# auggiemarignier/pxmcmc

Measured on AMD Instinct MI355X. Metric: MYULA samples/sec at L=256 synthesis, higher is better.
Workload: dtype f64

## Files before the change

pxmcmc_amd/csrc/sht_core.h:

```cpp
#pragma once
#include "common.h"

namespace pxm {

enum TableKind { TAB_INV = 0, TAB_FWD = 1, TAB_INV_ADJ = 2, TAB_FWD_ADJ = 3, TAB_GRAM = 4, TAB_GRAM_SPLIT = 5, TAB_KINDS = 6 };
inline bool kind_el_to_ring(int kind) { return kind == TAB_INV || kind == TAB_FWD_ADJ; }
inline bool kind_is_gram(int kind) { return kind == TAB_GRAM || kind == TAB_GRAM_SPLIT; }
inline bool kind_rows_are_el(int kind) { return kind == TAB_FWD || kind == TAB_INV_ADJ || kind_is_gram(kind); }
inline bool kind_k_is_el(int kind) { return kind == TAB_INV || kind == TAB_FWD_ADJ || kind_is_gram(kind); }

struct GemmTask {
  int64_t tab_off;
  int64_t rt_stride;
  int64_t x_off[4];
  int64_t y_off[4];
  int64_t x2_off[4];
  int64_t hd_off[4];
  int64_t ks_off[2];
  int64_t rs_off[2];
  int row_lo[2], row_hi[2];
  int k_beg, k_end;
  int row0;
  int n_rt;
  int nslab;
  double sign1;
  int m_unit;
  int hd_stride;
  int x_ncol, y_ncol;
};

struct GemmAffine {
  double ns = 0, wr = 0, wi = 0;
  int on = 0;
  int ncol_live = 1 << 30;
  uint64_t* bump = nullptr;
};

struct Profiler {
  struct Pool {
    std::vector<std::pair<hipEvent_t, hipEvent_t>> ev;
    size_t used = 0;
    double bytes = 0, flops = 0;
    std::vector<double> launch_bytes;
    std::vector<int> launch_wgs;
  };
  bool on = false;
  Pool gemm, dft;
  void next(Pool& p, hipEvent_t* start, hipEvent_t* stop, double alg_bytes, double flops, int workgroups = 0) {
    *start = *stop = nullptr;
    if (!on || p.used >= p.ev.size()) return;
    *start = p.ev[p.used].first;
// ... 9 lines not shown
int profiler_read(Profiler::Pool* p, double* ms, int64_t* launches, double* bytes, double* flops,
                  double* per_launch_ms = nullptr, double* per_launch_bytes = nullptr, int64_t cap = 0,
                  int32_t* per_launch_wgs = nullptr);
void profiler_release(Profiler* pr);

struct GemmFuse {
  int64_t x2_base = -1;
  const double* rscale = nullptr;
  int row_lo = 0, row_hi = 1 << 30;
  int64_t hd_base = -1;
  int hd_stride = 0;
};

struct ShtTables {
  int L = 0, spin = 0, Rp = 0;
  bool paired = false;
  int n_m = 0;
  double* d_tab[TAB_KINDS] = {};
  size_t bytes[TAB_KINDS] = {};
  std::vector<int64_t> m_off[TAB_KINDS];
  std::vector<int> k_beg[TAB_KINDS];
  std::vector<int64_t> odd_off;
  std::vector<int> odd_k_beg;
  int refs = 0;
  int m_of(int i) const { return paired ? i : i - (L - 1); }
};

inline bool gram_can_split(const ShtTables& T) { return T.paired && T.Rp % 32 == 0; }
constexpr int GEMM_TASK_FIXED_STEPS = 32;
inline int gram_half_k_beg(int m, int par) { return round_down((m - par + 1) / 2, 16); }
inline bool gram_order_splits(int Rp, int m) {
  auto work = [](int n, int kb) { return (n - kb) / 16 * (n - kb + GEMM_TASK_FIXED_STEPS); };
  return work(Rp / 2, gram_half_k_beg(m, 0)) + work(Rp / 2, gram_half_k_beg(m, 1)) < work(Rp, round_down(m, 16));
}

int get_tables(int L, int spin, unsigned kinds_mask, ShtTables** out);
void retain_tables(ShtTables* T);
void release_tables(ShtTables* T);
int64_t tables_trim();

void append_gemm_tasks(const ShtTables& T, int kind, int ncol, int64_t x_base, int x_L, int x_Rp,
                       int64_t y_base, int y_L, int y_Rp, const double* kscale, int64_t scratch_off,
                       const double* ws_base, std::vector<GemmTask>& tasks, int el_lo = 0,
                       const GemmFuse& fuse = GemmFuse());
struct GemmSide {
  int64_t x_base, y_base;
// ... 132 lines not shown
```

pxmcmc_amd/csrc/sht_gemm.hip:

```cpp
#include "../../include/pxmcmc_amd.h"
#include "sht_core.h"

#include <type_traits>

#include <hip/hip_ext.h>

#include <cstdlib>
#include <map>
#include <mutex>

namespace pxm {

typedef double d4 __attribute__((ext_vector_type(4)));

constexpr int KC = 16;
#define PXM_GEMM_MFMA(ACC, A, B) ACC = __builtin_amdgcn_mfma_f64_16x16x4f64(A, B, ACC, 0, 0, 0);
#ifdef PXM_GEMM_TRACE
__device__ unsigned long long* g_gemm_trace = nullptr;
extern "C" int pxm_debug_set_gemm_trace(unsigned long long* buf) {
  return hipMemcpyToSymbol(HIP_SYMBOL(g_gemm_trace), &buf, sizeof(buf)) == hipSuccess ? 0 : -1;
}
#endif
__device__ __forceinline__ double stage_add(double a, double b, bool on) { return a + (on ? b : 0.0); }
__device__ __forceinline__ double2 stage_add(double2 a, double2 b, bool on) { return double2{a.x + (on ? b.x : 0.0), a.y + (on ? b.y : 0.0)}; }
__device__ __forceinline__ double stage_scale(double a, double sc) { return a * sc; }
__device__ __forceinline__ double2 stage_scale(double2 a, double sc) { return double2{a.x * sc, a.y * sc}; }
template <int CT, int NSLAB>
struct GemmGeom {
  static constexpr int NCT = CT * NSLAB;
  static constexpr int COLS = 16 * NCT;
  static constexpr int PITCH = COLS + (COLS == 16 ? 0 : 16);
};
template <int CT, int NSLAB, int NW, int RT, int NSET, bool TWO, bool SK, int PK = 0>
__device__ __forceinline__ void sht_gemm_body(const GemmTask* __restrict__ tasks, const int bid,
                                              const double* __restrict__ X, double* __restrict__ Y, int ncol, int col0,
                                              const GemmAffine& aff, double (*xs)[KC][GemmGeom<CT, NSLAB>::PITCH]) {
  constexpr int NCT = CT * NSLAB;
  constexpr bool HOIST = TWO;
  constexpr int COLS = GemmGeom<CT, NSLAB>::COLS;
  constexpr int PITCH = GemmGeom<CT, NSLAB>::PITCH;
  constexpr int NT = 64 * NW;
  constexpr int VW = (KC * COLS / 2 >= NT) ? 2 : 1;
  constexpr int NV = KC * COLS / VW;
  constexpr int IT = (NV + NT - 1) / NT;
  const GemmTask t = tasks[bid];
  const int tid = threadIdx.x, lane = tid & 63;
  if (t.n_rt == 0) return;
  const int xn = (PK || TWO) ? t.x_ncol : ncol, yn = (PK || TWO) ? t.y_ncol : ncol;
#ifdef PXM_GEMM_TRACE
  const unsigned long long trace_t0 = wall_clock64();
  unsigned long long trace_t1 = 0, trace_t2 = 0;
  long long trace_c[5] = {0, 0, 0, 0, 0};
#define PXM_GEMM_CSTAMP(K) if (ch == 8) trace_c[K] = clock64();
#else
#define PXM_GEMM_CSTAMP(K)
#endif
// ... 128 lines not shown
  }
#undef PXM_STAGE_LOAD
#undef PXM_STAGE_STORE
#undef PXM_TAB_LOAD
#ifdef PXM_GEMM_TRACE
  trace_t2 = wall_clock64();
#endif

  constexpr int NGRP = PK ? 2 : 1;
  double hdv[RT][NSLAB][4], rsv[RT][NGRP][4];
#pragma unroll
  for (int r = 0; r < RT; ++r) {
    const int rowb = t.row0 + 16 * (r < n_my ? RT * wave + r : 0) + kq;
#pragma unroll
    for (int sl = 0; sl < NSLAB; ++sl)
#pragma unroll
      for (int q = 0; q < 4; ++q)
        hdv[r][sl][q] = (aff.on && t.hd_off[sl]) ? (X + t.hd_off[sl])[(int64_t)(rowb + 4 * q) * t.hd_stride + (cl & 1)] : 0.0;
#pragma unroll
    for (int g = 0; g < NGRP; ++g)
#pragma unroll
      for (int q = 0; q < 4; ++q) rsv[r][g][q] = t.rs_off[g] ? (X + t.rs_off[g])[rowb + 4 * q] : 1.0;
  }
  if constexpr (PK != 0) {
    const int slab = cl / PK, grp = slab >> 1;
    const bool live = slab < t.nslab;
    const double sgn = (slab & 1) ? t.sign1 : 1.0;
    const int64_t yo = tasks[bid].y_off[live ? slab : 0];
    const int row_lo = grp ? t.row_lo[1] : t.row_lo[0], row_hi = grp ? t.row_hi[1] : t.row_hi[0];
#pragma unroll
    for (int r = 0; r < RT; ++r) {
      if (r >= n_my) continue;
      const int rowb = t.row0 + 16 * (RT * wave + r) + kq;
      double* yb = Y + yo + col0 + (cl % PK) + (int64_t)rowb * yn;
#pragma unroll
      for (int q = 0; q < 4; ++q) {
        const int row = rowb + 4 * q;
        const double rs = grp ? rsv[r][NGRP - 1][q] : rsv[r][0][q];
        if (live && row >= row_lo && row < row_hi) yb[(int64_t)(4 * q) * yn] = sgn * rs * acc[r][0][q];
      }
    }
  } else {
#pragma unroll
  for (int r = 0; r < RT; ++r) {
    if (r >= n_my) continue;
#pragma unroll
// ... 21 lines not shown
  }
  }
#ifdef PXM_GEMM_TRACE
  __syncthreads();
  if (tid == 0 && g_gemm_trace) {
    unsigned hw, xcc;
    asm volatile("s_getreg_b32 %0, hwreg(HW_REG_HW_ID)" : "=s"(hw));
    asm volatile("s_getreg_b32 %0, hwreg(HW_REG_XCC_ID)" : "=s"(xcc));
    const unsigned long long slot = atomicAdd(g_gemm_trace, 1ull);
    unsigned long long* r = g_gemm_trace + 8 + 8 * slot;
    r[0] = blockIdx.x; r[1] = gridDim.x; r[2] = trace_t0; r[3] = wall_clock64();
    r[4] = ((unsigned long long)(xcc & 0xf) << 32) | hw; r[5] = (unsigned long long)nch | ((unsigned long long)t.n_rt << 16) | ((unsigned long long)aff.on << 32);
    r[6] = trace_t1; r[7] = trace_t2;
    if (nch > 9) {
      const unsigned long long s2 = atomicAdd(g_gemm_trace + 1, 1ull);
      unsigned long long* q = g_gemm_trace + 8 + 8 * 8192 + 8 * s2;
      q[0] = nch; q[1] = trace_c[1] - trace_c[0]; q[2] = trace_c[2] - trace_c[1]; q[3] = trace_c[3] - trace_c[2];
      q[4] = trace_c[4] - trace_c[3]; q[5] = aff.on; q[6] = gridDim.x; q[7] = 0;
    }
  }
#endif
}

template <int CT, int NSLAB, int NW, int RT, int NSET, bool TWO, bool SK>
__global__ __launch_bounds__(64 * NW) void k_sht_gemm(const GemmTask* __restrict__ tasks,
                                                      const double* __restrict__ X, double* __restrict__ Y,
                                                      int ncol, int col0, GemmAffine aff) {
  __shared__ double xs[2][KC][GemmGeom<CT, NSLAB>::PITCH];
  if (aff.bump && blockIdx.x == 0 && threadIdx.x == 0) *aff.bump += 1;
  sht_gemm_body<CT, NSLAB, NW, RT, NSET, TWO, SK>(tasks, blockIdx.x, X, Y, ncol, col0, aff, xs);
}
template <int PK, int NW, int RT, int NSET, bool TWO, bool SK>
__global__ __launch_bounds__(64 * NW) void k_sht_gemm_pk(const GemmTask* __restrict__ tasks, const double* __restrict__ X,
                                                         double* __restrict__ Y, int ncol, int col0, GemmAffine aff) {
  __shared__ double xs[2][KC][GemmGeom<1, 1>::PITCH];
  sht_gemm_body<1, 1, NW, RT, NSET, TWO, SK, PK>(tasks, blockIdx.x, X, Y, ncol, col0, aff, xs);
}

int profiler_enable(Profiler* pr, int max_launches) {
  profiler_release(pr);
  if (max_launches <= 0) return 0;
  for (Profiler::Pool* p : {&pr->gemm, &pr->dft}) {
    p->ev.resize((size_t)max_launches);
    for (auto& e : p->ev) {
      e.first = e.second = nullptr;
      PXM_HIP(hipEventCreate(&e.first));
      PXM_HIP(hipEventCreate(&e.second));
    }
  }
  pr->on = true;
  return 0;
}
void profiler_release(Profiler* pr) {
// ... 35 lines not shown
  return 0;
}

int check_gemm_task_ranges(const std::vector<GemmTask>& v, int nslab, int flags, int ncol, const double* ws_base,
                           const char* list_name) {
  int64_t n = 0;
  std::string why;
  auto bad = [&](size_t ti, const char* what, int col0) {
    set_error(std::string("GEMM task address range outside its buffer: list '") + list_name + "', task " + std::to_string(ti) +
              ", column group " + std::to_string(col0) + ", " + what + ": " + why);
    return -1;
  };
  auto ok = [&](int64_t lo, int64_t hi) {
    ++n;
    return lo <= hi && dev_range_ok(ws_base + lo, ws_base + hi + 1, &why);
  };
  const bool TWO = flags & 1, SK = flags & 2;
  for (size_t ti = 0; ti < v.size(); ++ti) {
    const GemmTask& t = v[ti];
    if (t.n_rt == 0) continue;
    const int nch = (t.k_end - t.k_beg) / KC;
    if (!ok(t.tab_off, t.tab_off + (int64_t)(t.n_rt - 1) * t.rt_stride + (int64_t)(2 * (nch - 1) + 1) * 128 + 127))
      return bad(ti, "ring-table stream", 0);
    for (int col0 = 0; col0 < ncol; col0 += 32) {
      const int CT = (ncol - col0 >= 32) ? 2 : 1;
      for (int slab = 0; slab < nslab; ++slab) {
        const int xn = ((TWO || nslab == 4) && t.x_ncol) ? t.x_ncol : ncol, yn = ((TWO || nslab == 4) && t.y_ncol) ? t.y_ncol : ncol;
        const int wx = std::min(16 * CT, xn), wy = std::min(16 * CT, yn);
        const int64_t lo = col0 + (int64_t)t.k_beg * xn, hi = col0 + wx - 1 + (int64_t)(t.k_end - 1) * xn;
        if (!ok(t.x_off[slab] + lo, t.x_off[slab] + hi)) return bad(ti, "operand staging", col0);
        if (TWO && t.x2_off[slab] && !ok(t.x2_off[slab] + lo, t.x2_off[slab] + hi)) return bad(ti, "second operand staging", col0);
        if (SK && t.ks_off[slab >> 1] && !ok(t.ks_off[slab >> 1] + t.k_beg, t.ks_off[slab >> 1] + t.k_end - 1))
          return bad(ti, "operand scale vector", col0);
        const int64_t r_lo = t.row0, r_hi = t.row0 + 16 * t.n_rt - 1;
        if (t.hd_off[slab] && !ok(t.hd_off[slab] + r_lo * t.hd_stride, t.hd_off[slab] + r_hi * t.hd_stride + 1))
          return bad(ti, "affine data term", col0);
        if (t.rs_off[slab >> 1] && !ok(t.rs_off[slab >> 1] + r_lo, t.rs_off[slab >> 1] + r_hi))
          return bad(ti, "per-row output scale", col0);
        const int64_t s_lo = std::max<int64_t>(r_lo, t.row_lo[slab >> 1]), s_hi = std::min<int64_t>(r_hi, (int64_t)t.row_hi[slab >> 1] - 1);
        if (s_lo <= s_hi && !ok(t.y_off[slab] + col0 + s_lo * yn, t.y_off[slab] + col0 + wy - 1 + s_hi * yn))
          return bad(ti, "result rows", col0);
      }
    }
  }
  ranges_checked_add(n);
  return 0;
}

int gemm_rows_per_task(int ncol) {
  (void)ncol;
  return 8;
}

int launch_gemm(const GemmTask* d_tasks, int n_tasks, int nslab, int flags, const double* X, double* Y, int ncol,
                int col0, int ct, double alg_bytes, double flops, hipStream_t stream, const GemmAffine& aff, Profiler* prof) {
  if (n_tasks == 0) return 0;
  PXM_REQUIRE(nslab == 1 || nslab == 2, "launch_gemm: nslab must be 1 (unpaired tables) or 2 (+-m pairs)");
  dim3 grid(n_tasks), block(512);
  hipEvent_t ev0 = nullptr, ev1 = nullptr;
  if (prof) prof->next(prof->gemm, &ev0, &ev1, alg_bytes, flops, n_tasks);
#define PXM_GEMM_L4(CT_, NS_, TWO_, SK_) \
  hipExtLaunchKernelGGL((k_sht_gemm<CT_, NS_, 8, 1, 2, TWO_, SK_>), grid, block, 0, stream, ev0, ev1, 0, d_tasks, X, Y, ncol, col0, aff)
#define PXM_GEMM_L3(CT_, NS_)                                   \
  switch (flags & 3) {                                          \
    case 0: PXM_GEMM_L4(CT_, NS_, false, false); break;         \
    case 1: PXM_GEMM_L4(CT_, NS_, true, false); break;          \
    case 2: PXM_GEMM_L4(CT_, NS_, false, true); break;          \
    default: PXM_GEMM_L4(CT_, NS_, true, true); break;          \
  }
  if (nslab == 2) {
    if (ct == 1) { PXM_GEMM_L3(1, 2) } else { PXM_GEMM_L3(2, 2) }
  } else {
    if (ct == 1) { PXM_GEMM_L3(1, 1) } else { PXM_GEMM_L3(2, 1) }
  }
#undef PXM_GEMM_L3
#undef PXM_GEMM_L4
  PXM_HIP(hipGetLastError());
  return 0;
}

int launch_gemm_packed(const GemmTask* d_tasks, int n_tasks, int pk, int flags, const double* X, double* Y, int ncol, int col0,
                       double alg_bytes, double flops, hipStream_t stream, Profiler* prof) {
  if (n_tasks == 0) return 0;
  PXM_REQUIRE(pk == 2 || pk == 4, "launch_gemm_packed: 2 or 4 live columns per slab");
  dim3 grid(n_tasks), block(512);
  hipEvent_t ev0 = nullptr, ev1 = nullptr;
  if (prof) prof->next(prof->gemm, &ev0, &ev1, alg_bytes, flops, n_tasks);
  GemmAffine aff;
#define PXM_PK_L(PK_, TWO_, SK_) \
  hipExtLaunchKernelGGL((k_sht_gemm_pk<PK_, 8, 1, 3, TWO_, SK_>), grid, block, 0, stream, ev0, ev1, 0, d_tasks, X, Y, ncol, col0, aff)
#define PXM_PK_N(PK_)                                     \
  switch (flags & 3) {                                    \
    case 0: PXM_PK_L(PK_, false, false); break;           \
// ... 26 lines not shown
    g.x_off[s1] = g.x_off[s0];
    g.y_off[s1] = g.y_off[s0];
  }
  g.ks_off[grp] = sd.kscale ? (sd.kscale - ws_base) : 0;
  g.rs_off[grp] = sd.fuse.rscale ? (sd.fuse.rscale - ws_base) : 0;
  g.row_lo[grp] = sd.fuse.row_lo;
  g.row_hi[grp] = sd.fuse.row_hi;
  g.x2_off[s0] = g.x2_off[s1] = 0;
  if (sd.fuse.x2_base >= 0) {
    g.x2_off[s0] = sd.fuse.x2_base + (int64_t)(m + sd.x_L - 1) * sd.x_Rp * xn;
    g.x2_off[s1] = (T.paired && m != 0) ? sd.fuse.x2_base + (int64_t)(-m + sd.x_L - 1) * sd.x_Rp * xn : g.x2_off[s0];
  }
  g.hd_off[s0] = g.hd_off[s1] = 0;
  g.hd_stride = sd.fuse.hd_stride > 0 ? sd.fuse.hd_stride : ncol;
  if (sd.fuse.hd_base >= 0) {
    g.hd_off[s0] = sd.fuse.hd_base + (int64_t)(m + sd.y_L - 1) * sd.y_Rp * g.hd_stride;
    g.hd_off[s1] = (T.paired && m != 0) ? sd.fuse.hd_base + (int64_t)(-m + sd.y_L - 1) * sd.y_Rp * g.hd_stride : g.hd_off[s0];
  }
  (void)kind;
}

static void append_block_tasks(const ShtTables& T, int kind, int ncol, const GemmSide& side, int64_t scratch_off,
                               const double* ws_base, std::vector<GemmTask>& tasks, int m, const double* tab, int kb, int n,
                               int par) {
  const bool rows_el = kind_rows_are_el(kind), k_el = kind_k_is_el(kind);
  const int lo16 = round_down(std::max(side.el_lo, 0), 16);
  const int rpt = gemm_rows_per_task(ncol);
  const int start = std::max(kb, lo16);
  if (start >= n) return;
  const int64_t rt_stride = (int64_t)((k_el ? n - kb : n) / 8) * 128;
  const int k_beg = k_el ? start : 0, k_end = n, row_beg = rows_el ? start : 0;
  const int64_t tab_skip = (rows_el ? (int64_t)((start - kb) / 16) * rt_stride : 0) + (k_el ? (int64_t)((start - kb) / 8) * 128 : 0);
  const int n_rt_total = (n - row_beg) / 16;
  for (int rt = 0; rt < n_rt_total; rt += rpt) {
    GemmTask g;
    g.m_unit = T.paired ? m : m + T.L - 1;
    g.tab_off = (tab + tab_skip + (int64_t)rt * rt_stride) - ws_base;
    g.rt_stride = rt_stride;
    for (int s = 0; s < 2; ++s) fill_side(g, s, T, kind, m, ncol, side, scratch_off, ws_base);
    g.nslab = T.paired ? 2 : 1;
    g.k_beg = k_beg;
    g.k_end = k_end;
    g.row0 = row_beg + 16 * rt;
    g.n_rt = std::min(rpt, n_rt_total - rt);
    g.sign1 = kind_is_gram(kind) ? 1.0 : ((m & 1) ? -1.0 : 1.0);
    g.x_ncol = side.x_ncol ? side.x_ncol : ncol;
    g.y_ncol = side.y_ncol ? side.y_ncol : ncol;
    if (par >= 0) {
      for (int s = 0; s < 4; ++s) {
        g.x_off[s] += par * g.x_ncol;
        g.y_off[s] += par * g.y_ncol;
        if (g.x2_off[s]) g.x2_off[s] += par * g.x_ncol;
        if (g.hd_off[s]) g.hd_off[s] += par * g.hd_stride;
      }
      g.x_ncol *= 2;
      g.y_ncol *= 2;
      g.hd_stride *= 2;
      for (int grp = 0; grp < 2; ++grp) g.row_lo[grp] = round_down(m, 16) / 2;
    }
    tasks.push_back(g);
  }
}

static void append_tasks_impl(const ShtTables& T, int kind, int ncol, const GemmSide& side,
                              int64_t scratch_off, const double* ws_base, std::vector<GemmTask>& tasks) {
  for (int i = 0; i < T.n_m; ++i) {
    const int m = T.m_of(i);
    const double* tab = T.d_tab[kind] + T.m_off[kind][i];
    const int kb = T.k_beg[kind][i];
    if (kind == TAB_GRAM_SPLIT && T.odd_off[i] >= 0) {
      append_block_tasks(T, kind, ncol, side, scratch_off, ws_base, tasks, m, tab, kb, T.Rp / 2, 0);
      append_block_tasks(T, kind, ncol, side, scratch_off, ws_base, tasks, m, T.d_tab[kind] + T.odd_off[i], T.odd_k_beg[i], T.Rp / 2, 1);
    } else {
      append_block_tasks(T, kind, ncol, side, scratch_off, ws_base, tasks, m, tab, kb, T.Rp, -1);
    }
  }
}

void append_gemm_tasks_packed(const ShtTables& T, int kind, int ncol, const GemmSide& side_a, const GemmSide* side_b,
                              int64_t scratch_off, const double* ws_base, std::vector<GemmTask>& tasks) {
  GemmSide sa = side_a;
  if (side_b) sa.el_lo = std::min(side_a.el_lo, side_b->el_lo);
  const size_t first = tasks.size();
  append_tasks_impl(T, kind, ncol, sa, scratch_off, ws_base, tasks);
  for (size_t i = first; i < tasks.size(); ++i) {
    GemmTask& g = tasks[i];
    const int m = T.paired ? g.m_unit : g.m_unit - (T.L - 1);
    fill_side(g, 0, T, kind, m, ncol, side_a, scratch_off, ws_base);
    fill_side(g, 1, T, kind, m, ncol, side_b ? *side_b : side_a, scratch_off, ws_base);
    g.nslab = side_b ? 4 : 2;
    g.x_ncol = side_a.x_ncol ? side_a.x_ncol : ncol;
    g.y_ncol = side_a.y_ncol ? side_a.y_ncol : ncol;
    if (!T.paired) {
// ... 19 lines not shown
  const double* Q = Qd + (int64_t)par * Rp * Rp;
  double acc = 0;
  for (int tp = 0; tp < L; ++tp) acc += B[(int64_t)tp * Rp + el] * Q[(int64_t)tp * Rp + t];
  Ad[(int64_t)i * Rp * Rp + (int64_t)el * Rp + t] = scale * acc;
}

__global__ void k_build_gram(const double* __restrict__ Bd, double* __restrict__ Gd, int Rp, int L) {
  const int i = blockIdx.z;
  const int r = blockIdx.x * 16 + threadIdx.x, c = blockIdx.y * 16 + threadIdx.y;
  const double* B = Bd + (int64_t)i * Rp * Rp;
  double acc = 0;
  for (int t = 0; t < L; ++t) acc += B[(int64_t)t * Rp + r] * B[(int64_t)t * Rp + c];
  Gd[(int64_t)i * Rp * Rp + (int64_t)r * Rp + c] = acc;
}

__global__ void k_tile_table(const double* __restrict__ D, double* __restrict__ out, int Rp, int n, int row_beg,
                             int k_beg, int transposed, int par) {
  const int nk2 = (n - k_beg) / 8;
  const int rt = blockIdx.y;
  const int kk2 = blockIdx.x;
  const int lane = threadIdx.x >> 1, h = threadIdx.x & 1;
  int row = row_beg + 16 * rt + (lane & 15);
  int k = k_beg + 8 * kk2 + 4 * h + (lane >> 4);
  if (par >= 0) {
    row = 2 * row + par;
    k = 2 * k + par;
  }
  const double v = transposed ? D[(int64_t)k * Rp + row] : D[(int64_t)row * Rp + k];
  out[((int64_t)rt * nk2 + kk2) * 128 + threadIdx.x] = v;
}

static std::mutex g_tab_mutex;
static std::map<std::pair<int, int>, ShtTables*> g_tab_cache;

static int build_gram_split(ShtTables& T, const double* d_G) {
  const int kind = TAB_GRAM_SPLIT, Rp = T.Rp, Rh = Rp / 2;
  PXM_REQUIRE(gram_can_split(T), "build_gram_split: the parity split needs spin-0 tables and Rp % 32 == 0");
  T.m_off[kind].assign(T.n_m, 0);
  T.k_beg[kind].assign(T.n_m, 0);
  T.odd_off.assign(T.n_m, -1);
  T.odd_k_beg.assign(T.n_m, 0);
  int64_t total = 0;
  for (int m = 0; m < T.n_m; ++m) {
    if (m == 0 || !gram_order_splits(Rp, m)) {
      const int kb = round_down(m, 16);
      T.k_beg[kind][m] = kb;
      T.m_off[kind][m] = total;
      total += (int64_t)((Rp - kb) / 16) * ((Rp - kb) / 8) * 128;
      continue;
    }
    for (int par = 0; par < 2; ++par) {
      const int kb = gram_half_k_beg(m, par);
      (par ? T.odd_k_beg[m] : T.k_beg[kind][m]) = kb;
      (par ? T.odd_off[m] : T.m_off[kind][m]) = total;
      total += (int64_t)((Rh - kb) / 16) * ((Rh - kb) / 8) * 128;
    }
  }
  T.bytes[kind] = (size_t)total * sizeof(double);
  if (int rc = dev_alloc(&T.d_tab[kind], T.bytes[kind], "ring table")) return rc;
  if (dry_run()) return 0;
  for (int m = 0; m < T.n_m; ++m) {
    const double* src = d_G + (int64_t)m * Rp * Rp;
    if (T.odd_off[m] < 0) {
      const int kb = T.k_beg[kind][m];
      hipLaunchKernelGGL(k_tile_table, dim3((Rp - kb) / 8, (Rp - kb) / 16), dim3(128), 0, 0, src, T.d_tab[kind] + T.m_off[kind][m],
                         Rp, Rp, kb, kb, 0, -1);
      continue;
    }
    for (int par = 0; par < 2; ++par) {
      const int kb = par ? T.odd_k_beg[m] : T.k_beg[kind][m];
      hipLaunchKernelGGL(k_tile_table, dim3((Rh - kb) / 8, (Rh - kb) / 16), dim3(128), 0, 0, src,
                         T.d_tab[kind] + (par ? T.odd_off[m] : T.m_off[kind][m]), Rp, Rh, kb, kb, 0, par);
    }
  }
  PXM_HIP(hipGetLastError());
  return 0;
}

static int build_kind(ShtTables& T, int kind, const double* d_B, const double* d_A, const double* d_G) {
  if (kind == TAB_GRAM_SPLIT) return build_gram_split(T, d_G);
  const int Rp = T.Rp;
  const bool rows_el = kind_rows_are_el(kind), k_el = kind_k_is_el(kind);
  T.m_off[kind].resize(T.n_m);
  T.k_beg[kind].resize(T.n_m);
  int64_t total = 0;
  for (int i = 0; i < T.n_m; ++i) {
    const int elmin = std::max(std::abs(T.m_of(i)), std::abs(T.spin));
    const int kb = round_down(elmin, 16);
    T.k_beg[kind][i] = kb;
    T.m_off[kind][i] = total;
    total += (int64_t)((rows_el ? Rp - kb : Rp) / 16) * ((k_el ? Rp - kb : Rp) / 8) * 128;
  }
  T.bytes[kind] = (size_t)total * sizeof(double);
  if (int rc = dev_alloc(&T.d_tab[kind], T.bytes[kind], "ring table")) return rc;
  if (dry_run()) return 0;
  for (int i = 0; i < T.n_m; ++i) {
    const int kb = T.k_beg[kind][i];
    const double* src;
    int transposed;
    if (kind == TAB_INV) { src = d_B; transposed = 0; }
    else if (kind == TAB_FWD_ADJ) { src = d_A; transposed = 1; }
    else if (kind == TAB_FWD) { src = d_A; transposed = 0; }
    else if (kind == TAB_INV_ADJ) { src = d_B; transposed = 1; }
// ... 40 lines not shown
      }
  } else if (missing) {
    const int Rp = T->Rp;
    const size_t dense = (size_t)T->n_m * Rp * Rp;
    std::vector<double> hB(dense, 0.0);
    const int m0 = T->paired ? 0 : -(L - 1);
    for (int i = 0; i < T->n_m; ++i) wigner_ring_table(L, spin, m0 + i, hB.data() + (size_t)i * Rp * Rp, Rp);
    double *d_B = nullptr, *d_A = nullptr, *d_Q = nullptr, *d_G = nullptr;
    PXM_HIP(hipMalloc(&d_B, dense * sizeof(double)));
    PXM_HIP(hipMemcpy(d_B, hB.data(), dense * sizeof(double), hipMemcpyHostToDevice));
    hB.clear();
    hB.shrink_to_fit();
    if (missing & ((1u << TAB_FWD) | (1u << TAB_FWD_ADJ))) {
      std::vector<double> hQ((size_t)2 * Rp * Rp, 0.0);
      quadrature_gram(L, +1, hQ.data(), Rp);
      quadrature_gram(L, -1, hQ.data() + (size_t)Rp * Rp, Rp);
      PXM_HIP(hipMalloc(&d_Q, hQ.size() * sizeof(double)));
      PXM_HIP(hipMemcpy(d_Q, hQ.data(), hQ.size() * sizeof(double), hipMemcpyHostToDevice));
      PXM_HIP(hipMalloc(&d_A, dense * sizeof(double)));
      dim3 grid(Rp / 16, Rp / 16, T->n_m), block(16, 16);
      hipLaunchKernelGGL(k_build_fwd, grid, block, 0, 0, d_B, d_Q, d_A, Rp, L, 2.0 * M_PI / (2 * L - 1), m0, spin);
      PXM_HIP(hipGetLastError());
    }
    if (missing & ((1u << TAB_GRAM) | (1u << TAB_GRAM_SPLIT))) {
      PXM_HIP(hipMalloc(&d_G, dense * sizeof(double)));
      dim3 grid(Rp / 16, Rp / 16, T->n_m), block(16, 16);
      hipLaunchKernelGGL(k_build_gram, grid, block, 0, 0, d_B, d_G, Rp, L);
      PXM_HIP(hipGetLastError());
    }
    for (int k = 0; k < TAB_KINDS; ++k)
      if (missing >> k & 1u) {
        int rc = build_kind(*T, k, d_B, d_A, d_G);
        if (rc) return rc;
      }
    PXM_HIP(hipDeviceSynchronize());
    PXM_HIP(hipFree(d_B));
    if (d_A) PXM_HIP(hipFree(d_A));
    if (d_Q) PXM_HIP(hipFree(d_Q));
    if (d_G) PXM_HIP(hipFree(d_G));
  }
  *out = T;
  return 0;
}

void retain_tables(ShtTables* T) {
  std::lock_guard<std::mutex> lock(g_tab_mutex);
  if (T) ++T->refs;
}
void release_tables(ShtTables* T) {
  std::lock_guard<std::mutex> lock(g_tab_mutex);
  if (T && T->refs > 0) --T->refs;
}
int64_t tables_trim() {
  std::lock_guard<std::mutex> lock(g_tab_mutex);
  int64_t freed = 0;
  for (auto it = g_tab_cache.begin(); it != g_tab_cache.end();) {
    ShtTables* T = it->second;
    if (T->refs > 0 || (dry_run() && it->first.first % 16 != 15)) {
      ++it;
      continue;
    }
    for (int k = 0; k < TAB_KINDS; ++k) {
      if (T->d_tab[k]) deferred_free(T->d_tab[k]);
      freed += (int64_t)T->bytes[k];
    }
    delete T;
    it = g_tab_cache.erase(it);
  }
  drain_deferred();
  return freed;
}

}
```

pxmcmc_amd/csrc/tasklist.h:

```cpp
#pragma once
#include "sht_core.h"

namespace pxm {

struct TaskList {
  GemmTask* d = nullptr;
  int n = 0;
  bool paired = false;
  int nslab = 2;
  std::vector<int> bls;
  std::vector<int> los;
  double mfma_units = 0;
  bool gram = false;
  double gram_table_bytes = 0;
  int flags = 0;
  int pk = 0;
  std::vector<char> tab_shared;
};

void order_tasks(std::vector<GemmTask>& v, const std::string& order);
int upload_tasks(std::vector<GemmTask> v, bool paired, TaskList* out, std::vector<int> bls, int ncol, const double* ws_base,
                 const char* name, std::vector<int> los = {}, int pk = 0, std::vector<char> tab_shared = {});
double tasklist_bytes(const TaskList& tl, int cg);
int run_tasks(const TaskList& tl, const double* X, double* Y, int ncol, int C, hipStream_t st,
              const GemmAffine& aff = GemmAffine(), Profiler* prof = nullptr);
void free_tasks(TaskList* t);

}
```

pxmcmc_amd/csrc/tasklist.hip:

```cpp
#include "tasklist.h"

#include <algorithm>
#include <cstdlib>
#include <cstring>
#include <map>

namespace pxm {

static int64_t task_work(const GemmTask& a, int64_t fixed) { return (int64_t)(a.k_end - a.k_beg + fixed) * a.n_rt; }

static void order_xcd(std::vector<GemmTask>& v, int64_t fixed) {
  constexpr int NQ = 8;
  std::map<int64_t, int> unit_of;
  std::vector<std::vector<GemmTask>> units;
  for (const GemmTask& t : v) {
    auto it = unit_of.find(t.x_off[0]);
    if (it == unit_of.end()) {
      it = unit_of.emplace(t.x_off[0], (int)units.size()).first;
      units.emplace_back();
    }
    units[it->second].push_back(t);
  }
  std::vector<int64_t> uw(units.size(), 0);
  std::vector<int> idx(units.size());
// ... 32 lines not shown
  std::vector<std::vector<GemmTask>> bins(nbins);
  std::vector<int64_t> load(nbins, 0);
  for (const GemmTask& t : v) {
    int best = 0;
    for (int b = 1; b < nbins; ++b)
      if (load[b] < load[best] || (load[b] == load[best] && bins[b].size() < bins[best].size())) best = b;
    bins[best].push_back(t);
    load[best] += task_work(t, fixed);
  }
  std::vector<GemmTask> ordered;
  ordered.reserve(v.size());
  for (size_t r = 0;; ++r) {
    bool any = false;
    for (int b = 0; b < nbins; ++b)
      if (r < bins[b].size()) {
        ordered.push_back(bins[b][r]);
        any = true;
      }
    if (!any) break;
  }
  v.swap(ordered);
}

void order_tasks(std::vector<GemmTask>& v, const std::string& order) {
  const int64_t fixed = order == "xcd" ? GEMM_TASK_FIXED_STEPS : 0;
  std::stable_sort(v.begin(), v.end(), [&](const GemmTask& a, const GemmTask& b) { return task_work(a, fixed) > task_work(b, fixed); });
  if (order == "xcd" && !v.empty()) order_xcd(v, fixed);
  else if (order == "bins" && (int)v.size() > 256) order_bins(v, fixed);
}

int upload_tasks(std::vector<GemmTask> v, bool paired, TaskList* out, std::vector<int> bls, int ncol, const double* ws_base,
                 const char* name, std::vector<int> los, int pk, std::vector<char> tab_shared) {
  tab_shared.resize(bls.size(), 0);
  los.resize(bls.size(), 0);
  out->pk = pk;
  out->tab_shared = tab_shared;
  out->bls = bls;
  out->los = los;
  const char* order_env = getenv("PXM_GEMM_ORDER");
  order_tasks(v, order_env ? order_env : (v.size() > 2048 ? "xcd" : "bins"));
  out->n = (int)v.size();
  out->paired = paired;
  out->nslab = pk ? 4 : (paired ? 2 : 1);
  for (const GemmTask& t : v) {
    PXM_REQUIRE(t.n_rt >= 0 && t.n_rt <= 8 && t.row0 >= 0 && t.row0 % 16 == 0 && t.k_beg >= 0 && t.k_beg % 16 == 0 &&
                    (t.n_rt == 0 || (t.k_end > t.k_beg && (t.k_end - t.k_beg) % 16 == 0)),
                "upload_tasks: malformed GEMM task");
    out->mfma_units += (double)t.n_rt * ((t.k_end - t.k_beg) / 4) * (pk ? 1 : t.nslab);
    for (int sl = 0; sl < 4; ++sl)
      if (t.x2_off[sl]) out->flags |= 1;
    if (t.ks_off[0] || t.ks_off[1]) out->flags |= 2;
  }
  if (!pk && !(out->flags & 1))
    for (const GemmTask& t : v)
      PXM_REQUIRE(t.n_rt == 0 || (t.x_ncol == ncol && t.y_ncol == ncol), "upload_tasks: a streaming list with a row pitch of its own");
  if (v.empty()) return 0;
  if (int rc = check_gemm_task_ranges(v, out->nslab, out->flags, ncol, ws_base, name)) return rc;
  if (int rc = dev_alloc(&out->d, v.size() * sizeof(GemmTask), "GEMM task list")) return rc;
  return dev_upload(out->d, v.data(), v.size() * sizeof(GemmTask));
}

double tasklist_bytes(const TaskList& tl, int cg) {
  double bytes = 0;
  for (size_t i = 0; i < tl.bls.size(); ++i) {
    const double Ld = tl.bls[i];
    if (tl.gram) bytes += tl.gram_table_bytes + 3 * 16.0 * cg * Ld * Ld + 16.0 * Ld * Ld;
    else bytes += gemm_alg_bytes(tl.bls[i], tl.paired, cg, tl.los[i]);
    if (!tl.gram && tl.pk && tl.tab_shared[i]) bytes -= gemm_table_bytes(tl.bls[i], tl.paired, tl.los[i]);
  }
  return bytes;
}

int run_tasks(const TaskList& tl, const double* X, double* Y, int ncol, int C, hipStream_t st, const GemmAffine& aff,
              Profiler* prof) {
  note_stream(st);
  if (tl.pk)
    return launch_gemm_packed(tl.d, tl.n, tl.pk, tl.flags, X, Y, ncol, 0, tasklist_bytes(tl, C), tl.mfma_units * 2048.0, st, prof);
  for (int col0 = 0; col0 < ncol; col0 += 32) {
    const int ct = (ncol - col0 >= 32) ? 2 : 1;
    const int cg = std::max(0, std::min(C - col0 / 2, 8 * ct));
    if (cg == 0) break;
    const double bytes = tasklist_bytes(tl, cg);
    GemmAffine a = aff;
    if (col0) a.bump = nullptr;
    a.ncol_live = 2 * C;
    int rc = launch_gemm(tl.d, tl.n, tl.nslab, tl.flags, X, Y, ncol, col0, ct, bytes, tl.mfma_units * ct * 2048.0, st, a, prof);
    if (rc) return rc;
  }
  return 0;
// ... 9 lines not shown
```

pxmcmc_amd/csrc/wav_plan.hip:

```cpp
#include "wav_plan.h"

#include <cmath>
#include <memory>
#include <mutex>

using namespace pxm;

struct SideOverride {
  const int64_t* g = nullptr;
  int g_ncol = 0;
  const WlAttach* h = nullptr;
};
static GemmSide wav_side(const pxm_wav_plan_s* p, int s, int which, const SideOverride& ov = SideOverride()) {
  const int L = p->L, b = p->bl[s], Rb = round_up(b, 16);
  const int64_t G = ov.g ? *ov.g : p->offG[s];
  GemmSide g;
  const bool ring_is_x = which == 0 || which == 3;
  if (ov.g && ov.g_ncol) (ring_is_x ? g.x_ncol : g.y_ncol) = ov.g_ncol;
  if (ov.h) (ring_is_x ? g.y_ncol : g.x_ncol) = ov.h->ncol_h;
  g.el_lo = p->el_lo_s[s];
  g.fuse = GemmFuse();
  g.kscale = nullptr;
  const int cls = (s == 0) ? 1 : ((s - 1) & 1);
  const int64_t hcls = ov.h ? (cls ? ov.h->offHBn : ov.h->offHAn) : (cls ? p->offHB : p->offHA);
// ... 170 lines not shown
  if ((rc = wav_level_list(p, TAB_FWD_ADJ, p->offHA, p->offGL, sum2, &p->anadj_fwdadj, "analysis-adjoint forward-adjoint at L"))) return rc;
  p->lane_of.assign(p->nsc, -1);
  SidePool* sp = nullptr;
  if ((rc = side_pool(&sp))) return rc;
  for (int i = 0; i < p->nside; ++i) {
    p->side[i] = sp->side[i];
    p->ev_join[i] = sp->ev_join[i];
  }
  p->ev_fork = sp->ev_fork;
  int k = 0;
  for (int s = p->nsc - 1; s >= 0; --s)
    if (p->bl[s] < L) p->lane_of[s] = (k++) % p->nside;
  std::vector<const DftPlan*> dp;
  for (int s = 0; s < p->nsc; ++s) dp.push_back(&p->dft[s]);
  if ((rc = dft_group_create(dp, p->offG, p->coef_off, p->ncol, p->ws, &p->dft_group)) < 0) return rc;
  *plan = guard.release();
  return 0;
}

int pxm::wav_make_gram_lists(pxm_wav_plan_s* p) {
  if (p->gram.d) return 0;
  int rc;
  const char* split_env = getenv("PXM_GRAM_SPLIT");
  const int kind = (gram_can_split(*p->TL) && !(split_env && atoi(split_env) == 0)) ? TAB_GRAM_SPLIT : TAB_GRAM;
  if ((rc = get_tables(p->L, p->spin, 1u << kind, &p->TL))) return rc;
  wav_hold(p, p->TL);
  std::vector<GemmTask> v;
  GemmFuse fz;
  fz.x2_base = p->offHB;
  fz.hd_base = p->offHDc;
  fz.hd_stride = 2;
  append_gemm_tasks(*p->TL, kind, p->ncol, p->offHA, p->L, p->Rp, p->offHL, p->L, p->Rp, nullptr, p->offS, p->ws, v, 0, fz);
  if ((rc = upload_tasks(v, p->TL->paired, &p->gram, {p->L}, p->ncol, p->ws, "Gram step"))) return rc;
  p->gram.gram = true;
  p->gram.gram_table_bytes = (double)p->TL->bytes[kind];
  return wav_level_list(p, TAB_INV_ADJ, p->offGD, p->offHD, GemmFuse(), &p->adj_invadj_D, "inverse-adjoint of the data rings");
}

namespace pxm {
__global__ void k_iter_add(uint64_t* c, uint64_t inc) { *c += inc; }

__global__ void k_count_nonfinite(const double* __restrict__ x, int64_t n, unsigned long long* cnt) {
  unsigned long long c = 0;
  for (int64_t i = blockIdx.x * (int64_t)blockDim.x + threadIdx.x; i < n; i += (int64_t)gridDim.x * blockDim.x)
    if (!isfinite(x[i])) ++c;
  if (c) atomicAdd(cnt, c);
}
}

extern "C" {

int pxm_wav_plan_create(int L, double B, int J_min, int max_chains, unsigned flags, pxm_wav_plan_t* plan) {
  (void)flags;
  return wav_plan_create_impl("pxm_wav_plan_create", L, B, J_min, 0, max_chains, plan);
}

int pxm_wav_plan_create_spin(int L, double B, int J_min, int spin, int max_chains, unsigned flags, pxm_wav_plan_t* plan) {
  (void)flags;
// ... 139 lines not shown
```

Baseline: 117,600.

## Split order-0 Gram block by parity with a rank-one pole correction

Adds a TAB_GRAM_SPLIT0 table kind and makes it the default. It splits the m=0 Gram block into even and odd halves, as already done for other orders. The cross-parity coupling from the pole ring is handled as a rank-one correction computed inside the GEMM kernel through a new POLE template path. This is meant to halve the dense order-0 table stream and its MFMA work. In exchange it adds an in-kernel reduction with extra syncthreads, a new kernel instantiation for the Gram list, and a dependence on the coupling being exactly rank one.

```diff
diff --git a/pxmcmc_amd/csrc/sht_core.h b/pxmcmc_amd/csrc/sht_core.h
--- a/pxmcmc_amd/csrc/sht_core.h
+++ b/pxmcmc_amd/csrc/sht_core.h
@@ -3,9 +3,10 @@
 
 namespace pxm {
 
-enum TableKind { TAB_INV = 0, TAB_FWD = 1, TAB_INV_ADJ = 2, TAB_FWD_ADJ = 3, TAB_GRAM = 4, TAB_GRAM_SPLIT = 5, TAB_KINDS = 6 };
+enum TableKind { TAB_INV = 0, TAB_FWD = 1, TAB_INV_ADJ = 2, TAB_FWD_ADJ = 3, TAB_GRAM = 4, TAB_GRAM_SPLIT = 5, TAB_GRAM_SPLIT0 = 6, TAB_KINDS = 7 };
 inline bool kind_el_to_ring(int kind) { return kind == TAB_INV || kind == TAB_FWD_ADJ; }
-inline bool kind_is_gram(int kind) { return kind == TAB_GRAM || kind == TAB_GRAM_SPLIT; }
+inline bool kind_is_gram_split(int kind) { return kind == TAB_GRAM_SPLIT || kind == TAB_GRAM_SPLIT0; }
+inline bool kind_is_gram(int kind) { return kind == TAB_GRAM || kind_is_gram_split(kind); }
 inline bool kind_rows_are_el(int kind) { return kind == TAB_FWD || kind == TAB_INV_ADJ || kind_is_gram(kind); }
 inline bool kind_k_is_el(int kind) { return kind == TAB_INV || kind == TAB_FWD_ADJ || kind_is_gram(kind); }
 
@@ -27,6 +28,10 @@
   int m_unit;
   int hd_stride;
   int x_ncol, y_ncol;
+  int pole_n;
+  int pole_dx;
+  int64_t pole_b_off;
+  int64_t pole_bo_off;
 };
 
 struct GemmAffine {
@@ -82,6 +87,7 @@
   std::vector<int> k_beg[TAB_KINDS];
   std::vector<int64_t> odd_off;
   std::vector<int> odd_k_beg;
+  double* d_pole = nullptr;
   int refs = 0;
   int m_of(int i) const { return paired ? i : i - (L - 1); }
 };
diff --git a/pxmcmc_amd/csrc/sht_gemm.hip b/pxmcmc_amd/csrc/sht_gemm.hip
--- a/pxmcmc_amd/csrc/sht_gemm.hip
+++ b/pxmcmc_amd/csrc/sht_gemm.hip
@@ -31,7 +31,7 @@
   static constexpr int COLS = 16 * NCT;
   static constexpr int PITCH = COLS + (COLS == 16 ? 0 : 16);
 };
-template <int CT, int NSLAB, int NW, int RT, int NSET, bool TWO, bool SK, int PK = 0>
+template <int CT, int NSLAB, int NW, int RT, int NSET, bool TWO, bool SK, int PK = 0, bool POLE = false>
 __device__ __forceinline__ void sht_gemm_body(const GemmTask* __restrict__ tasks, const int bid,
                                               const double* __restrict__ X, double* __restrict__ Y, int ncol, int col0,
                                               const GemmAffine& aff, double (*xs)[KC][GemmGeom<CT, NSLAB>::PITCH]) {
@@ -206,6 +206,53 @@
 #pragma unroll
       for (int q = 0; q < 4; ++q) rsv[r][g][q] = t.rs_off[g] ? (X + t.rs_off[g])[rowb + 4 * q] : 1.0;
   }
+  if constexpr (POLE) {
+    if (t.pole_n) {
+      constexpr int W2 = 8 * CT;
+      constexpr int NRG = NT / W2;
+      const int cp = tid % W2, rg = tid / W2;
+      const double* xo = X + t.x_off[0] + t.pole_dx + col0 + 2 * cp;
+      const double* xo2 = two ? X + t.x2_off[0] + t.pole_dx + col0 + 2 * cp : xo;
+      const double* bo = X + t.pole_bo_off;
+      double bown[RT][4];
+#pragma unroll
+      for (int r = 0; r < RT; ++r)
+#pragma unroll
+        for (int q = 0; q < 4; ++q)
+          bown[r][q] = (X + t.pole_b_off)[t.row0 + 16 * (r < n_my ? RT * wave + r : 0) + kq + 4 * q];
+      double2 part{0.0, 0.0};
+#pragma unroll 1
+      for (int r = rg; r < t.pole_n; r += NRG) {
+        const double2 a = *reinterpret_cast<const double2*>(xo + (int64_t)r * xn);
+        const double2 a2 = *reinterpret_cast<const double2*>(xo2 + (int64_t)r * xn);
+        const double bv = bo[r];
+        const double2 v = stage_add(a, a2, two);
+        part.x += bv * v.x;
+        part.y += bv * v.y;
+      }
+#pragma unroll
+      for (int msk = W2; msk < 64; msk <<= 1) {
+        part.x += __shfl_xor(part.x, msk);
+        part.y += __shfl_xor(part.y, msk);
+      }
+      double* red = &xs[0][0][0];
+      __syncthreads();
+      if (lane < W2) *reinterpret_cast<double2*>(red + wave * 2 * W2 + 2 * lane) = part;
+      __syncthreads();
+#pragma unroll
+      for (int ct = 0; ct < CT; ++ct) {
+        double sc = 0.0;
+#pragma unroll
+        for (int w = 0; w < NW; ++w) sc += red[w * 2 * W2 + 16 * ct + cl];
+#pragma unroll
+        for (int r = 0; r < RT; ++r)
+#pragma unroll
+          for (int sl = 0; sl < NSLAB; ++sl)
+#pragma unroll
+            for (int q = 0; q < 4; ++q) acc[r][sl * CT + ct][q] += 0.5 * bown[r][q] * sc;
+      }
+    }
+  }
   if constexpr (PK != 0) {
     const int slab = cl / PK, grp = slab >> 1;
     const bool live = slab < t.nslab;
@@ -273,13 +320,14 @@
 #endif
 }
 
-template <int CT, int NSLAB, int NW, int RT, int NSET, bool TWO, bool SK>
+template <int CT, int NSLAB, int NW, int RT, int NSET, bool TWO, bool SK, bool POLE = false>
 __global__ __launch_bounds__(64 * NW) void k_sht_gemm(const GemmTask* __restrict__ tasks,
                                                       const double* __restrict__ X, double* __restrict__ Y,
                                                       int ncol, int col0, GemmAffine aff) {
   __shared__ double xs[2][KC][GemmGeom<CT, NSLAB>::PITCH];
+  static_assert(!POLE || 2 * KC * GemmGeom<CT, NSLAB>::PITCH >= NW * 16 * CT, "the pole reduction borrows the operand buffers");
   if (aff.bump && blockIdx.x == 0 && threadIdx.x == 0) *aff.bump += 1;
-  sht_gemm_body<CT, NSLAB, NW, RT, NSET, TWO, SK>(tasks, blockIdx.x, X, Y, ncol, col0, aff, xs);
+  sht_gemm_body<CT, NSLAB, NW, RT, NSET, TWO, SK, 0, POLE>(tasks, blockIdx.x, X, Y, ncol, col0, aff, xs);
 }
 template <int PK, int NW, int RT, int NSET, bool TWO, bool SK>
 __global__ __launch_bounds__(64 * NW) void k_sht_gemm_pk(const GemmTask* __restrict__ tasks, const double* __restrict__ X,
@@ -361,6 +409,14 @@
     const int nch = (t.k_end - t.k_beg) / KC;
     if (!ok(t.tab_off, t.tab_off + (int64_t)(t.n_rt - 1) * t.rt_stride + (int64_t)(2 * (nch - 1) + 1) * 128 + 127))
       return bad(ti, "ring-table stream", 0);
+    for (int col0 = 0; col0 < ncol && t.pole_n; col0 += 32) {
+      const int CT = (ncol - col0 >= 32) ? 2 : 1;
+      if (!ok(t.pole_b_off + t.row0, t.pole_b_off + t.row0 + 16 * t.n_rt - 1)) return bad(ti, "pole column of the task's rows", col0);
+      if (!ok(t.pole_bo_off, t.pole_bo_off + t.pole_n - 1)) return bad(ti, "pole column of the other parity", col0);
+      const int64_t lo = t.pole_dx + col0, hi = t.pole_dx + col0 + 16 * CT - 1 + (int64_t)(t.pole_n - 1) * t.x_ncol;
+      if (!ok(t.x_off[0] + lo, t.x_off[0] + hi)) return bad(ti, "pole term operand", col0);
+      if (t.x2_off[0] && !ok(t.x2_off[0] + lo, t.x2_off[0] + hi)) return bad(ti, "pole term second operand", col0);
+    }
     for (int col0 = 0; col0 < ncol; col0 += 32) {
       const int CT = (ncol - col0 >= 32) ? 2 : 1;
       for (int slab = 0; slab < nslab; ++slab) {
@@ -407,7 +463,11 @@
     case 2: PXM_GEMM_L4(CT_, NS_, false, true); break;          \
     default: PXM_GEMM_L4(CT_, NS_, true, true); break;          \
   }
-  if (nslab == 2) {
+  if (flags & 4) {
+    PXM_REQUIRE(nslab == 2 && (flags & 3) == 1, "launch_gemm: a pole term outside the Gram list");
+    if (ct == 1) hipExtLaunchKernelGGL((k_sht_gemm<1, 2, 8, 1, 2, true, false, true>), grid, block, 0, stream, ev0, ev1, 0, d_tasks, X, Y, ncol, col0, aff);
+    else hipExtLaunchKernelGGL((k_sht_gemm<2, 2, 8, 1, 2, true, false, true>), grid, block, 0, stream, ev0, ev1, 0, d_tasks, X, Y, ncol, col0, aff);
+  } else if (nslab == 2) {
     if (ct == 1) { PXM_GEMM_L3(1, 2) } else { PXM_GEMM_L3(2, 2) }
   } else {
     if (ct == 1) { PXM_GEMM_L3(1, 1) } else { PXM_GEMM_L3(2, 1) }
@@ -480,13 +540,13 @@
 
 static void append_block_tasks(const ShtTables& T, int kind, int ncol, const GemmSide& side, int64_t scratch_off,
                                const double* ws_base, std::vector<GemmTask>& tasks, int m, const double* tab, int kb, int n,
-                               int par) {
+                               int par, int64_t rt_stride_stored = 0, const double* pole = nullptr) {
   const bool rows_el = kind_rows_are_el(kind), k_el = kind_k_is_el(kind);
   const int lo16 = round_down(std::max(side.el_lo, 0), 16);
   const int rpt = gemm_rows_per_task(ncol);
   const int start = std::max(kb, lo16);
   if (start >= n) return;
-  const int64_t rt_stride = (int64_t)((k_el ? n - kb : n) / 8) * 128;
+  const int64_t rt_stride = rt_stride_stored ? rt_stride_stored : (int64_t)((k_el ? n - kb : n) / 8) * 128;
   const int k_beg = k_el ? start : 0, k_end = n, row_beg = rows_el ? start : 0;
   const int64_t tab_skip = (rows_el ? (int64_t)((start - kb) / 16) * rt_stride : 0) + (k_el ? (int64_t)((start - kb) / 8) * 128 : 0);
   const int n_rt_total = (n - row_beg) / 16;
@@ -504,6 +564,14 @@
     g.sign1 = kind_is_gram(kind) ? 1.0 : ((m & 1) ? -1.0 : 1.0);
     g.x_ncol = side.x_ncol ? side.x_ncol : ncol;
     g.y_ncol = side.y_ncol ? side.y_ncol : ncol;
+    g.pole_n = g.pole_dx = 0;
+    g.pole_b_off = g.pole_bo_off = 0;
+    if (pole) {
+      g.pole_n = n;
+      g.pole_dx = par ? -g.x_ncol : g.x_ncol;
+      g.pole_b_off = (pole + par * n) - ws_base;
+      g.pole_bo_off = (pole + (1 - par) * n) - ws_base;
+    }
     if (par >= 0) {
       for (int s = 0; s < 4; ++s) {
         g.x_off[s] += par * g.x_ncol;
@@ -526,7 +594,12 @@
     const int m = T.m_of(i);
     const double* tab = T.d_tab[kind] + T.m_off[kind][i];
     const int kb = T.k_beg[kind][i];
-    if (kind == TAB_GRAM_SPLIT && T.odd_off[i] >= 0) {
+    if (kind == TAB_GRAM_SPLIT0 && m == 0) {
+      const int Rh = T.Rp / 2;
+      const int64_t rs = (int64_t)(T.Rp / 8) * 128;
+      append_block_tasks(T, kind, ncol, side, scratch_off, ws_base, tasks, m, tab, 0, Rh, 0, rs, T.d_pole);
+      append_block_tasks(T, kind, ncol, side, scratch_off, ws_base, tasks, m, tab + (Rh / 16) * rs + (int64_t)(Rh / 8) * 128, 0, Rh, 1, rs, T.d_pole);
+    } else if (kind_is_gram_split(kind) && T.odd_off[i] >= 0) {
       append_block_tasks(T, kind, ncol, side, scratch_off, ws_base, tasks, m, tab, kb, T.Rp / 2, 0);
       append_block_tasks(T, kind, ncol, side, scratch_off, ws_base, tasks, m, T.d_tab[kind] + T.odd_off[i], T.odd_k_beg[i], T.Rp / 2, 1);
     } else {
@@ -592,7 +665,10 @@
   const int lane = threadIdx.x >> 1, h = threadIdx.x & 1;
   int row = row_beg + 16 * rt + (lane & 15);
   int k = k_beg + 8 * kk2 + 4 * h + (lane >> 4);
-  if (par >= 0) {
+  if (par == 2) {
+    row = row < n / 2 ? 2 * row : 2 * (row - n / 2) + 1;
+    k = k < n / 2 ? 2 * k : 2 * (k - n / 2) + 1;
+  } else if (par >= 0) {
     row = 2 * row + par;
     k = 2 * k + par;
   }
@@ -603,8 +679,8 @@
 static std::mutex g_tab_mutex;
 static std::map<std::pair<int, int>, ShtTables*> g_tab_cache;
 
-static int build_gram_split(ShtTables& T, const double* d_G) {
-  const int kind = TAB_GRAM_SPLIT, Rp = T.Rp, Rh = Rp / 2;
+static int build_gram_split(ShtTables& T, int kind, const double* d_G) {
+  const int Rp = T.Rp, Rh = Rp / 2;
   PXM_REQUIRE(gram_can_split(T), "build_gram_split: the parity split needs spin-0 tables and Rp % 32 == 0");
   T.m_off[kind].assign(T.n_m, 0);
   T.k_beg[kind].assign(T.n_m, 0);
@@ -628,13 +704,22 @@
   }
   T.bytes[kind] = (size_t)total * sizeof(double);
   if (int rc = dev_alloc(&T.d_tab[kind], T.bytes[kind], "ring table")) return rc;
+  if (kind == TAB_GRAM_SPLIT0 && !T.d_pole) {
+    if (int rc = dev_alloc(&T.d_pole, (size_t)Rp * sizeof(double), "pole column of the order-0 Gram block")) return rc;
+    if (!dry_run()) {
+      std::vector<double> B0((size_t)Rp * Rp, 0.0), b(Rp, 0.0);
+      wigner_ring_table(T.L, 0, 0, B0.data(), Rp);
+      for (int l = 0; l < T.L; ++l) b[(l & 1) * Rh + l / 2] = B0[(size_t)(T.L - 1) * Rp + l];
+      if (int rc = dev_upload(T.d_pole, b.data(), b.size() * sizeof(double))) return rc;
+    }
+  }
   if (dry_run()) return 0;
   for (int m = 0; m < T.n_m; ++m) {
     const double* src = d_G + (int64_t)m * Rp * Rp;
     if (T.odd_off[m] < 0) {
       const int kb = T.k_beg[kind][m];
       hipLaunchKernelGGL(k_tile_table, dim3((Rp - kb) / 8, (Rp - kb) / 16), dim3(128), 0, 0, src, T.d_tab[kind] + T.m_off[kind][m],
-                         Rp, Rp, kb, kb, 0, -1);
+                         Rp, Rp, kb, kb, 0, (kind == TAB_GRAM_SPLIT0 && m == 0) ? 2 : -1);
       continue;
     }
     for (int par = 0; par < 2; ++par) {
@@ -648,7 +733,7 @@
 }
 
 static int build_kind(ShtTables& T, int kind, const double* d_B, const double* d_A, const double* d_G) {
-  if (kind == TAB_GRAM_SPLIT) return build_gram_split(T, d_G);
+  if (kind_is_gram_split(kind)) return build_gram_split(T, kind, d_G);
   const int Rp = T.Rp;
   const bool rows_el = kind_rows_are_el(kind), k_el = kind_k_is_el(kind);
   T.m_off[kind].resize(T.n_m);
@@ -735,7 +820,7 @@
       hipLaunchKernelGGL(k_build_fwd, grid, block, 0, 0, d_B, d_Q, d_A, Rp, L, 2.0 * M_PI / (2 * L - 1), m0, spin);
       PXM_HIP(hipGetLastError());
     }
-    if (missing & ((1u << TAB_GRAM) | (1u << TAB_GRAM_SPLIT))) {
+    if (missing & ((1u << TAB_GRAM) | (1u << TAB_GRAM_SPLIT) | (1u << TAB_GRAM_SPLIT0))) {
       PXM_HIP(hipMalloc(&d_G, dense * sizeof(double)));
       dim3 grid(Rp / 16, Rp / 16, T->n_m), block(16, 16);
       hipLaunchKernelGGL(k_build_gram, grid, block, 0, 0, d_B, d_G, Rp, L);
@@ -777,6 +862,7 @@
       if (T->d_tab[k]) deferred_free(T->d_tab[k]);
       freed += (int64_t)T->bytes[k];
     }
+    if (T->d_pole) deferred_free(T->d_pole);
     delete T;
     it = g_tab_cache.erase(it);
   }
diff --git a/pxmcmc_amd/csrc/tasklist.h b/pxmcmc_amd/csrc/tasklist.h
--- a/pxmcmc_amd/csrc/tasklist.h
+++ b/pxmcmc_amd/csrc/tasklist.h
@@ -13,6 +13,8 @@
   double mfma_units = 0;
   bool gram = false;
   double gram_table_bytes = 0;
+  bool gram_pole = false;
+  double gram_stream_bytes = 0;
   int flags = 0;
   int pk = 0;
   std::vector<char> tab_shared;
diff --git a/pxmcmc_amd/csrc/tasklist.hip b/pxmcmc_amd/csrc/tasklist.hip
--- a/pxmcmc_amd/csrc/tasklist.hip
+++ b/pxmcmc_amd/csrc/tasklist.hip
@@ -78,8 +78,11 @@
   v.swap(ordered);
 }
 
+#ifndef PXM_BINS_FIXED_STEPS
+#define PXM_BINS_FIXED_STEPS GEMM_TASK_FIXED_STEPS
+#endif
 void order_tasks(std::vector<GemmTask>& v, const std::string& order) {
-  const int64_t fixed = order == "xcd" ? GEMM_TASK_FIXED_STEPS : 0;
+  const int64_t fixed = order == "xcd" ? GEMM_TASK_FIXED_STEPS : PXM_BINS_FIXED_STEPS;
   std::stable_sort(v.begin(), v.end(), [&](const GemmTask& a, const GemmTask& b) { return task_work(a, fixed) > task_work(b, fixed); });
   if (order == "xcd" && !v.empty()) order_xcd(v, fixed);
   else if (order == "bins" && (int)v.size() > 256) order_bins(v, fixed);
@@ -106,6 +109,7 @@
     for (int sl = 0; sl < 4; ++sl)
       if (t.x2_off[sl]) out->flags |= 1;
     if (t.ks_off[0] || t.ks_off[1]) out->flags |= 2;
+    if (t.pole_n) out->flags |= 4;
   }
   if (!pk && !(out->flags & 1))
     for (const GemmTask& t : v)
@@ -120,7 +124,8 @@
   double bytes = 0;
   for (size_t i = 0; i < tl.bls.size(); ++i) {
     const double Ld = tl.bls[i];
-    if (tl.gram) bytes += tl.gram_table_bytes + 3 * 16.0 * cg * Ld * Ld + 16.0 * Ld * Ld;
+    if (tl.gram) bytes += (tl.gram_pole ? tl.gram_stream_bytes + 2 * 2 * 16.0 * cg * Ld + 2 * 2 * 8.0 * Ld : tl.gram_table_bytes) +
+                          3 * 16.0 * cg * Ld * Ld + 16.0 * Ld * Ld;
     else bytes += gemm_alg_bytes(tl.bls[i], tl.paired, cg, tl.los[i]);
     if (!tl.gram && tl.pk && tl.tab_shared[i]) bytes -= gemm_table_bytes(tl.bls[i], tl.paired, tl.los[i]);
   }
diff --git a/pxmcmc_amd/csrc/wav_plan.hip b/pxmcmc_amd/csrc/wav_plan.hip
--- a/pxmcmc_amd/csrc/wav_plan.hip
+++ b/pxmcmc_amd/csrc/wav_plan.hip
@@ -216,7 +216,8 @@
   if (p->gram.d) return 0;
   int rc;
   const char* split_env = getenv("PXM_GRAM_SPLIT");
-  const int kind = (gram_can_split(*p->TL) && !(split_env && atoi(split_env) == 0)) ? TAB_GRAM_SPLIT : TAB_GRAM;
+  const int split = split_env ? atoi(split_env) : 2;
+  const int kind = (!gram_can_split(*p->TL) || split == 0) ? TAB_GRAM : (split == 1 ? TAB_GRAM_SPLIT : TAB_GRAM_SPLIT0);
   if ((rc = get_tables(p->L, p->spin, 1u << kind, &p->TL))) return rc;
   wav_hold(p, p->TL);
   std::vector<GemmTask> v;
@@ -228,6 +229,8 @@
   if ((rc = upload_tasks(v, p->TL->paired, &p->gram, {p->L}, p->ncol, p->ws, "Gram step"))) return rc;
   p->gram.gram = true;
   p->gram.gram_table_bytes = (double)p->TL->bytes[kind];
+  p->gram.gram_pole = kind == TAB_GRAM_SPLIT0;
+  p->gram.gram_stream_bytes = p->gram.gram_table_bytes - (p->gram.gram_pole ? 4.0 * p->Rp * p->Rp : 0.0);
   return wav_level_list(p, TAB_INV_ADJ, p->offGD, p->offHD, GemmFuse(), &p->adj_invadj_D, "inverse-adjoint of the data rings");
 }
 
```

Result: faster. 121,700, median of 6 (+3.5%).
